# psweens/VAN-GAN

Hardware: AMD Instinct MI355X
Metric: train Mvoxels/s (VanGan.train_step, 128^3 bf16) (higher is better)
Workload: dtype bf16; 1 GPU; VanGan.train_step, 128x128x128 volumes, batch 1 per GPU (global 1), clDice on, disc noise+dropout on; parallelism=dp1

## Files before the change

van_gan_amd/csrc/vg_c1k3.hip:

```cpp
#include "vg_c1k3.h"

namespace {
constexpr int TW = 16, TD = 4;
constexpr int ROWB = TW * 8 + 8;

typedef __attribute__((ext_vector_type(2))) unsigned u32x2;
typedef __attribute__((ext_vector_type(4))) unsigned u32x4;
typedef __attribute__((ext_vector_type(4))) short s16x4;
typedef __attribute__((ext_vector_type(2))) float f32x2;

template <int KS, int ST, int TH> struct Geo {
    static constexpr int IH = ST * TH + KS - ST, ID = ST * TD + KS - ST;
    static constexpr int NROWS = ID * IH, IMGB = NROWS * ROWB;
    static constexpr int NI = 3 * ST + 4;
    static constexpr int NRT = KS * KS;
};

__device__ __forceinline__ float c1_slope(int act) { return act == VG_ACT_RELU ? 0.f : (act == VG_ACT_LRELU ? VG_LRELU : 1.f); }

template <typename S, int KS, int ST, int TH, bool NOISE>
__device__ __forceinline__ void c1_stage_image(const C1M& p, char* img, int n, int od0, int oh0, int ow0, float sc, float sf, float slope, int tid) {
    typedef Geo<KS, ST, TH> G;
    const bool refl = p.pad_mode == VG_PAD_REFLECT;
    for (int item = tid; item < G::NROWS * 4; item += 256) {
        const int row = item >> 2, q = item & 3;
        const int zz = row / G::IH, yy = row - zz * G::IH;
        const int pd = ST * od0 + p.td0 + zz, ph = ST * oh0 + p.th0 + yy, pw0 = ST * (ow0 + 4 * q) + p.tw0;
        bool okd, okh;
        const int rd = c1_resolve(pd, p.D, refl, okd), rh = c1_resolve(ph, p.H, refl, okh);
        const S* src = (const S*)p.x + (((int64_t)n * p.D + rd) * p.H + rh) * p.W;
        const bf16_t* nz = nullptr;
        if (NOISE) nz = (const bf16_t*)p.noise + (((int64_t)n * (p.D + 2) + min(max(pd + 1, 0), p.D + 1)) * (p.H + 2) + min(max(ph + 1, 0), p.H + 1)) * (p.W + 2);
        float v[G::NI], nv[G::NI]; bool ok[G::NI];
#pragma unroll
        for (int i = 0; i < G::NI; ++i) {
            const int cw = c1_resolve(pw0 + i, p.W, refl, ok[i]);
            v[i] = ld_global(src + cw);
            nv[i] = NOISE ? ld_global(nz + min(max(pw0 + i + 1, 0), p.W + 1)) : 0.f;
        }
        unsigned short h[G::NI];
#pragma unroll
        for (int i = 0; i < G::NI; ++i) {
            float y = v[i] * sc + sf;
            y = fmaxf(y, y * slope);
            y = (okd && okh && ok[i]) ? y : 0.f;
            h[i] = f2bf(y + nv[i]);
        }
        char* dst = img + row * ROWB + q * 32;
#pragma unroll
        for (int e = 0; e < 4; ++e)
            *(u32x2*)(dst + e * 8) = (u32x2){h[ST * e] | ((unsigned)h[ST * e + 1] << 16), h[ST * e + 2] | ((unsigned)h[ST * e + 3] << 16)};
    }
}

template <int KS>
__device__ __forceinline__ bf16x8 c1_weight_frag(const C1M& p, int co, int kg, int s) {
    bf16x8 r;
#pragma unroll
    for (int i = 0; i < 8; ++i) {
        const int k = 32 * s + 8 * kg + i, t = k >> 2, j = k & 3;
        r[i] = (t < KS * KS && j < KS) ? (short)((const bf16_t*)p.w)[(size_t)co * p.Ktot + t * p.CK + j] : (short)0;
    }
    return r;
}

template <typename S, int KS, int ST, int MT, bool NOISE>
__global__ __launch_bounds__(256, 2) void c1m_fwd_kernel(const C1M p) {
    typedef bf16_t T;
    constexpr int TH = 8, C = 16 * MT;
    typedef Geo<KS, ST, TH> G;
    __shared__ __attribute__((aligned(16))) char img[G::IMGB];
    __shared__ float stat[32 * MT];
    const int tid = threadIdx.x, lane = tid & 63, wave = __builtin_amdgcn_readfirstlane(tid >> 6);
    const int li = lane & 15, kg = lane >> 4;
    const int n = blockIdx.y;
    const float sc = p.scale ? p.scale[n] : p.sc, sf = p.scale ? p.shift[n] : p.sf, slope = c1_slope(p.act);
    bf16x8 wa[MT][2];
    f32x2 eb[MT][2];
#pragma unroll
    for (int mt = 0; mt < MT; ++mt) {
        wa[mt][0] = c1_weight_frag<KS>(p, 16 * mt + li, kg, 0); wa[mt][1] = c1_weight_frag<KS>(p, 16 * mt + li, kg, 1);
        const int c = 16 * mt + 4 * kg;
        eb[mt][0] = (f32x2){0.f, 0.f}; eb[mt][1] = eb[mt][0];
        if (p.bias) { eb[mt][0] = (f32x2){p.bias[c], p.bias[c + 1]}; eb[mt][1] = (f32x2){p.bias[c + 2], p.bias[c + 3]}; }
    }
    if (tid < 32 * MT) stat[tid] = 0.f;
    int boff[2][2];
#pragma unroll
    for (int s = 0; s < 2; ++s)
#pragma unroll
        for (int h = 0; h < 2; ++h) {
            const int t = min(8 * s + 2 * kg + h, G::NRT - 1), a = t / KS, b = t - a * KS;
            boff[s][h] = ((ST * wave + a) * G::IH + b) * ROWB + li * 8;
        }
    const int tiles_w = (p.OW + TW - 1) / TW, tiles_h = (p.OH + TH - 1) / TH, tiles_d = (p.OD + TD - 1) / TD;
    const int ntiles = tiles_w * tiles_h * tiles_d;
    float s1[MT][4], s2[MT][4];
#pragma unroll
    for (int mt = 0; mt < MT; ++mt)
#pragma unroll
        for (int r = 0; r < 4; ++r) { s1[mt][r] = 0.f; s2[mt][r] = 0.f; }
    const int cst = 8 * (kg >> 1), jodd = kg & 1;
    const size_t rowpitch = (size_t)p.OW * C;
    for (int tile = blockIdx.x; tile < ntiles; tile += gridDim.x) {
        const int tw = tile % tiles_w, t2 = tile / tiles_w, th = t2 % tiles_h, td = t2 / tiles_h;
        const int od0 = td * TD, oh0 = th * TH, ow0 = tw * TW;
        __syncthreads();
        c1_stage_image<S, KS, ST, TH, NOISE>(p, img, n, od0, oh0, ow0, sc, sf, slope, tid);
        __syncthreads();
        const int od = od0 + wave, ow = ow0 + li;
        const bool dw_ok = od < p.OD && ow < p.OW;
        T* const obase = (T*)p.out + ((((size_t)n * p.OD + min(od, p.OD - 1)) * p.OH + oh0) * p.OW + min(ow, p.OW - 1)) * C + cst;
#pragma unroll
        for (int mt = 0; mt < MT; ++mt) {
            f32x4 acc[8];
#pragma unroll
            for (int j = 0; j < 8; ++j) {
                const int jo = ST * j * ROWB;
                const u32x2 a0 = *(const u32x2*)(img + boff[0][0] + jo), a1 = *(const u32x2*)(img + boff[0][1] + jo);
                const u32x2 c0 = *(const u32x2*)(img + boff[1][0] + jo), c1 = *(const u32x2*)(img + boff[1][1] + jo);
                const bf16x8 b0 = __builtin_bit_cast(bf16x8, ((u32x4){a0[0], a0[1], a1[0], a1[1]}));
                const bf16x8 b1 = __builtin_bit_cast(bf16x8, ((u32x4){c0[0], c0[1], c1[0], c1[1]}));
                acc[j] = VG_MFMA16(wa[mt][0], b0, ((f32x4){0.f, 0.f, 0.f, 0.f}));
                acc[j] = VG_MFMA16(wa[mt][1], b1, acc[j]);
            }
            T* const optr = obase + 16 * mt;
#pragma unroll
            for (int jp = 0; jp < 8; jp += 2) {
                bf16x4 pk[2];
#pragma unroll
                for (int e = 0; e < 2; ++e) {
                    const int j = jp + e;
                    const bool ok = dw_ok && oh0 + j < p.OH;
                    f32x2 v0 = {acc[j][0], acc[j][1]}, v1 = {acc[j][2], acc[j][3]};
                    v0 += eb[mt][0]; v1 += eb[mt][1];
                    pk[e] = (bf16x4){(short)f2bf(v0[0]), (short)f2bf(v0[1]), (short)f2bf(v1[0]), (short)f2bf(v1[1])};
                    f32x2 q0 = {bf2f((bf16_t)pk[e][0]), bf2f((bf16_t)pk[e][1])}, q1 = {bf2f((bf16_t)pk[e][2]), bf2f((bf16_t)pk[e][3])};
                    if (!ok) { q0 = (f32x2){0.f, 0.f}; q1 = q0; }
                    s1[mt][0] += q0[0]; s1[mt][1] += q0[1]; s1[mt][2] += q1[0]; s1[mt][3] += q1[1];
                    s2[mt][0] += q0[0] * q0[0]; s2[mt][1] += q0[1] * q0[1]; s2[mt][2] += q1[0] * q1[0]; s2[mt][3] += q1[1] * q1[1];
                }
                const u32x2 wa_ = __builtin_bit_cast(u32x2, pk[0]), wb_ = __builtin_bit_cast(u32x2, pk[1]);
                const u32x2 x0 = __builtin_amdgcn_permlane16_swap(wa_[0], wb_[0], false, false);
                const u32x2 x1 = __builtin_amdgcn_permlane16_swap(wa_[1], wb_[1], false, false);
                const u32x4 outv = {x0[0], x1[0], x0[1], x1[1]};
                const int j = jp + jodd;
                if (dw_ok && oh0 + j < p.OH) *(u32x4*)(optr + j * rowpitch) = outv;
            }
        }
    }
    if (!p.sums) return;
#pragma unroll
    for (int mt = 0; mt < MT; ++mt)
#pragma unroll
        for (int r = 0; r < 4; ++r) {
            float a = s1[mt][r], b = s2[mt][r];
#pragma unroll
            for (int o = 1; o < 16; o <<= 1) { a += __shfl_xor(a, o); b += __shfl_xor(b, o); }
            if (li == 0) { atomicAdd(&stat[(16 * mt + 4 * kg + r) * 2], a); atomicAdd(&stat[(16 * mt + 4 * kg + r) * 2 + 1], b); }
        }
    __syncthreads();
    if (tid < 32 * MT) {
        const int stripe = blockIdx.x & (VG_STRIPES - 1);
        atomicAdd(&p.sums[((size_t)stripe * gridDim.y + n) * (2 * C) + tid], stat[tid]);
    }
    if (p.fin.ticket) vg_fin_tail(p.fin, p.sums, gridDim.y, C, gridDim.x * gridDim.y, (int*)img);
}

template <typename S, int KS, int ST, int TH, int NT, bool NOISE>
__global__ __launch_bounds__(256, 2) void c1m_wgrad_kernel(const C1M p) {
    typedef bf16_t T;
    typedef Geo<KS, ST, TH> G;
    constexpr int C = 16 * NT, VB = 2 * C;
    constexpr int DYROW = TW * VB, DYB = TD * TH * DYROW;
    constexpr int MTS = (G::NRT + 1 + 3) / 4;
    constexpr int UPT = DYB / 16 / 256;
    static_assert(MTS * NT * 1024 <= DYB, "the accumulator exchange reuses the dY tile");
    __shared__ __attribute__((aligned(16))) char img[G::IMGB + 16];
    __shared__ __attribute__((aligned(16))) char dyt[DYB];
    const int tid = threadIdx.x, lane = tid & 63, wave = __builtin_amdgcn_readfirstlane(tid >> 6);
    const int n = blockIdx.y;
    const float sc = p.scale ? p.scale[n] : p.sc, sf = p.scale ? p.shift[n] : p.sf, slope = c1_slope(p.act);
    if (tid == 0) {
        const unsigned one = f2bf(1.f);
        *(u32x4*)(img + G::IMGB) = (u32x4){one | (one << 16), one | (one << 16), 0u, 0u};
    }
    const int g = lane >> 4, q = (lane >> 2) & 3, pp = lane & 3;
    const int wq = 8 * (g & 1) + q, yq = g >> 1;
    int aoff[MTS], amove[MTS];
#pragma unroll
    for (int mt = 0; mt < MTS; ++mt) {
        const int r = 4 * mt + pp, a = r / KS, b = r - a * KS;
        amove[mt] = r < G::NRT ? 1 : 0;
        aoff[mt] = r < G::NRT ? ((ST * wave + a) * G::IH + ST * yq + b) * ROWB + wq * 8 : (r == G::NRT ? G::IMGB : G::IMGB + 8);
    }
    const int boff = ((wave * TH + yq) * TW + wq) * VB + pp * 8;
    const int tiles_w = (p.OW + TW - 1) / TW, tiles_h = (p.OH + TH - 1) / TH, tiles_d = (p.OD + TD - 1) / TD;
    const int ntiles = tiles_w * tiles_h * tiles_d;
    f32x4 acc[MTS][NT];
#pragma unroll
    for (int mt = 0; mt < MTS; ++mt)
#pragma unroll
        for (int nt = 0; nt < NT; ++nt) acc[mt][nt] = (f32x4){0.f, 0.f, 0.f, 0.f};
    typedef __attribute__((address_space(3))) s16x4 lds_s4;
    for (int tile = blockIdx.x; tile < ntiles; tile += gridDim.x) {
        const int tw = tile % tiles_w, t2 = tile / tiles_w, th = t2 % tiles_h, td = t2 / tiles_h;
        const int od0 = td * TD, oh0 = th * TH, ow0 = tw * TW;
        f32x4 dv[UPT];
#pragma unroll
        for (int i = 0; i < UPT; ++i) {
            const int u = tid + 256 * i, vox = u / (2 * NT), c16 = u - vox * (2 * NT);
            const int w = vox & 15, y = (vox >> 4) % TH, z = vox / (16 * TH);
            const bool ok = od0 + z < p.OD && oh0 + y < p.OH && ow0 + w < p.OW;
            const T* src = (const T*)p.dy + ((((size_t)n * p.OD + min(od0 + z, p.OD - 1)) * p.OH + min(oh0 + y, p.OH - 1)) * p.OW + min(ow0 + w, p.OW - 1)) * C + c16 * 8;
            dv[i] = *(const __attribute__((address_space(1))) f32x4*)(uintptr_t)src;
            if (!ok) dv[i] = (f32x4){0.f, 0.f, 0.f, 0.f};
        }
        __syncthreads();
        c1_stage_image<S, KS, ST, TH, NOISE>(p, img, n, od0, oh0, ow0, sc, sf, slope, tid);
#pragma unroll
        for (int i = 0; i < UPT; ++i) *(f32x4*)(dyt + (tid + 256 * i) * 16) = dv[i];
        __syncthreads();
#pragma unroll
        for (int s = 0; s < TH / 2; ++s) {
            bf16x8 a[MTS];
#pragma unroll
            for (int mt = 0; mt < MTS; ++mt) {
                const int o = aoff[mt] + amove[mt] * (s * 2 * ST * ROWB);
                const s16x4 lo = __builtin_amdgcn_ds_read_tr16_b64_v4i16((lds_s4*)(img + o));
                const s16x4 hi = __builtin_amdgcn_ds_read_tr16_b64_v4i16((lds_s4*)(img + o + amove[mt] * 32));
                a[mt] = (bf16x8){lo[0], lo[1], lo[2], lo[3], hi[0], hi[1], hi[2], hi[3]};
            }
#pragma unroll
            for (int nt = 0; nt < NT; ++nt) {
                const s16x4 lo = __builtin_amdgcn_ds_read_tr16_b64_v4i16((lds_s4*)(dyt + boff + s * 2 * DYROW + nt * 32));
                const s16x4 hi = __builtin_amdgcn_ds_read_tr16_b64_v4i16((lds_s4*)(dyt + boff + s * 2 * DYROW + nt * 32 + 4 * VB));
                const bf16x8 b = {lo[0], lo[1], lo[2], lo[3], hi[0], hi[1], hi[2], hi[3]};
#pragma unroll
                for (int mt = 0; mt < MTS; ++mt) acc[mt][nt] = VG_MFMA16(a[mt], b, acc[mt][nt]);
            }
        }
    }
    float* red = (float*)dyt;
    __syncthreads();
    for (int i = tid; i < MTS * NT * 256; i += 256) red[i] = 0.f;
    __syncthreads();
#pragma unroll
    for (int mt = 0; mt < MTS; ++mt)
#pragma unroll
        for (int nt = 0; nt < NT; ++nt)
#pragma unroll
            for (int e = 0; e < 4; ++e) atomicAdd(&red[((mt * NT + nt) * 4 + e) * 64 + lane], acc[mt][nt][e]);
    __syncthreads();
    float* slab = p.part ? p.part + ((size_t)blockIdx.y * gridDim.x + blockIdx.x) * (KS * KS * KS * C) : nullptr;
    for (int i = tid; i < MTS * NT * 256; i += 256) {
        const int l = i & 63, e = (i >> 6) & 3, t = i >> 8, nt = t % NT, mt = t / NT;
        const int r = 4 * mt + (l >> 4), co = 16 * nt + (l & 15);
        const float v = red[i];
        if (r < G::NRT && e < KS) {
            const int idx = (r * KS + e) * C + co;
            if (slab) slab[idx] = v; else atomicAdd(&p.dw[idx], v);
        } else if (r == G::NRT && e == 0 && p.db) atomicAdd(&p.db[co], v);
    }
}
}

static bool c1m_fill(const vg_conv_desc* d, C1M& p) {
    if (!vg_tune("C1M", 1) || d->f32 || d->out_f32 || d->c_src0 != 1 || d->src1 || d->c_src1 || d->nclass > 1) return false;
    const int KS = d->wpack;
    if (KS != 3 && KS != 4) return false;
    if (d->istr != KS - 2 || d->ntaps != KS * KS || d->Cout != (KS == 3 ? 16 : 64)) return false;
    for (int t = 0; t < KS * KS; ++t)
        if (d->tap_d[t] != d->tap_d[0] + t / KS || d->tap_h[t] != d->tap_h[0] + t % KS || d->tap_w[t] != 0) return false;
    if (d->noise && !(d->noise_pad == 1 && d->pad_mode == VG_PAD_REFLECT)) return false;
    if (d->D < 2 || d->H < 2 || d->W < 2 || d->OD < 1 || d->OH < 1 || d->OW < 1) return false;
    p = C1M{};
    p.x = d->src0; p.x_f32 = d->src_f32; p.sc = 1.f; p.sf = 0.f; p.scale = d->in_scale; p.shift = d->in_shift; p.act = d->act;
    p.pad_mode = d->pad_mode; p.noise = d->noise;
    p.D = d->D; p.H = d->H; p.W = d->W; p.OD = d->OD; p.OH = d->OH; p.OW = d->OW; p.C = d->Cout;
    p.td0 = d->tap_d[0]; p.th0 = d->tap_h[0]; p.tw0 = d->wpack_wmin;
    p.w = d->wpacked; p.CK = d->CK; p.Ktot = ((KS * KS * d->CK + 31) / 32) * 32;
    return true;
}
static dim3 c1m_grid(const C1M& c, int N, int th, int per_cu) {
    const int64_t tiles = (int64_t)((c.OD + TD - 1) / TD) * ((c.OH + th - 1) / th) * ((c.OW + TW - 1) / TW);
    int64_t b = (int64_t)256 * per_cu / (N > 0 ? N : 1);
    if (b > tiles) b = tiles;
    if (b < 1) b = 1;
    return dim3((unsigned)b, (unsigned)N);
}

template <typename S, int KS, int MT>
static void c1m_launch_fwd(const C1M& c, dim3 grid, hipStream_t s) {
    if (c.noise) hipLaunchKernelGGL((c1m_fwd_kernel<S, KS, KS - 2, MT, true>), grid, dim3(256), 0, s, c);
    else hipLaunchKernelGGL((c1m_fwd_kernel<S, KS, KS - 2, MT, false>), grid, dim3(256), 0, s, c);
}
int c1m_fwd(const vg_conv_desc* d, hipStream_t s) {
    C1M c;
    if (!c1m_fill(d, c)) return 1;
    c.bias = d->bias; c.out = d->out; c.sums = d->out_sums; c.fin = vg_fin_of(d);
    const int KS = d->wpack;
    if (vg_dry("c1m_fwd<%s,%d,%d,%d,n%d>", d->src_f32 ? "f32" : "bf16", KS, KS - 2, c.C / 16, c.noise ? 1 : 0)) return VG_OK;
    const dim3 grid = c1m_grid(c, d->N, 8, vg_tune("C1M_FWD_WGS", KS == 3 ? 4 : 2));
    if (KS == 3) { if (d->src_f32) c1m_launch_fwd<float, 3, 1>(c, grid, s); else c1m_launch_fwd<bf16_t, 3, 1>(c, grid, s); }
    else { if (d->src_f32) c1m_launch_fwd<float, 4, 4>(c, grid, s); else c1m_launch_fwd<bf16_t, 4, 4>(c, grid, s); }
    if (c.sums && c.fin.ticket) vg_fin_done = true;
    return vg_check_launch();
}

template <typename S, int KS, int TH, int NT>
static void c1m_launch_wgrad(const C1M& c, dim3 grid, hipStream_t s) {
    if (c.noise) hipLaunchKernelGGL((c1m_wgrad_kernel<S, KS, KS - 2, TH, NT, true>), grid, dim3(256), 0, s, c);
    else hipLaunchKernelGGL((c1m_wgrad_kernel<S, KS, KS - 2, TH, NT, false>), grid, dim3(256), 0, s, c);
}
int c1m_wgrad(const vg_conv_desc* d, const void* dy, int dy_f32, int T_total, float* dw, float* db, float* scratch, int64_t scratch_bytes, hipStream_t s) {
    C1M c;
    if (dy_f32 || !vg_tune("C1M_WGRAD", 1) || !c1m_fill(d, c)) return 1;
    const int KS = d->wpack;
    if (T_total != KS * KS) return 1;
    c.dy = dy; c.dw = dw; c.db = db;
    const int th = KS == 3 ? 8 : 4;
    const dim3 grid = c1m_grid(c, d->N, th, vg_tune("C1M_WGRAD_WGS", KS == 3 ? 2 : 1));
    const int nslab = (int)(grid.x * grid.y), dw_elems = KS * KS * KS * c.C;
    c.part = (nslab > 4 && scratch && (int64_t)nslab * dw_elems * 4 <= scratch_bytes && vg_tune("C1M_WGRAD_PART", 1)) ? scratch : nullptr;
    if (vg_dry("c1m_wgrad<%s,%d,%d,%d,n%d>|part%d", d->src_f32 ? "f32" : "bf16", KS, KS - 2, c.C / 16, c.noise ? 1 : 0, c.part ? 1 : 0)) return VG_OK;
    if (KS == 3) { if (d->src_f32) c1m_launch_wgrad<float, 3, 8, 1>(c, grid, s); else c1m_launch_wgrad<bf16_t, 3, 8, 1>(c, grid, s); }
    else { if (d->src_f32) c1m_launch_wgrad<float, 4, 4, 4>(c, grid, s); else c1m_launch_wgrad<bf16_t, 4, 4, 4>(c, grid, s); }
    if (c.part) vg_launch_reduce_partials(c.part, nslab, dw_elems, dw, s);
    return vg_check_launch();
}

namespace {
__global__ __launch_bounds__(256) void cell_pack_kernel(const float* __restrict__ w, int C, int Ktot, bf16_t* __restrict__ out) {
    const size_t total = (size_t)64 * Ktot;
    for (size_t i = (size_t)blockIdx.x * 256 + threadIdx.x; i < total; i += (size_t)gridDim.x * 256) {
        const int row = (int)(i / Ktot), k = (int)(i % Ktot);
        const int chunk = k / 448, kl = k % 448, tap = kl / 16, ch = chunk * 16 + (kl & 15);
        float v = 0.f;
        if (row < 8 && tap < 27 && ch < C) {
            const int nd = tap / 9, nh = (tap / 3) % 3, nw = tap % 3;
            const int td = ((row >> 2) & 1) + 2 - 2 * nd, th = ((row >> 1) & 1) + 2 - 2 * nh, tw = (row & 1) + 2 - 2 * nw;
            if (td >= 0 && th >= 0 && tw >= 0) v = w[(size_t)((td * 4 + th) * 4 + tw) * C + ch];
        }
        out[i] = f2bf(v);
    }
}
__global__ __launch_bounds__(256) void cells_fold_kernel(const bf16_t* __restrict__ cells, int D, int H, int W, float* __restrict__ dx) {
    const int n = blockIdx.y;
    const int CD = D / 2 + 1, CH = H / 2 + 1, CW = W / 2 + 1;
    const bf16_t* cb = cells + (size_t)n * CD * CH * CW * 16;
    const int64_t total = (int64_t)D * H * W;
    for (int64_t i = (int64_t)blockIdx.x * 256 + threadIdx.x; i < total; i += (int64_t)gridDim.x * 256) {
        const int iw = (int)(i % W); const int64_t r = i / W; const int ih = (int)(r % H), id = (int)(r / H);
        int pd[2], ph[2], pw[2], nd = 1, nh = 1, nw = 1;
        pd[0] = id + 1; ph[0] = ih + 1; pw[0] = iw + 1;
        if (id == 1) pd[nd++] = 0; else if (id == D - 2) pd[nd++] = D + 1;
        if (ih == 1) ph[nh++] = 0; else if (ih == H - 2) ph[nh++] = H + 1;
        if (iw == 1) pw[nw++] = 0; else if (iw == W - 2) pw[nw++] = W + 1;
        float s = 0.f;
        for (int a = 0; a < nd; ++a)
            for (int b = 0; b < nh; ++b)
                for (int c = 0; c < nw; ++c) {
                    const int qd = pd[a], qh = ph[b], qw = pw[c];
                    s += bf2f(cb[(((size_t)(qd >> 1) * CH + (qh >> 1)) * CW + (qw >> 1)) * 16 + ((qd & 1) * 4 + (qh & 1) * 2 + (qw & 1))]);
                }
        dx[(size_t)n * total + i] = s;
    }
}
}

extern "C" int vg_pack_cell_weights(const float* w, int C, void* out, vg_stream_t stream) {
    vg_begin();
    if (!w || !out || C < 16 || (C % 16)) return VG_EINVAL;
    const int Ktot = (C / 16) * 448;
    hipLaunchKernelGGL(cell_pack_kernel, dim3((64 * Ktot + 255) / 256), dim3(256), 0, (hipStream_t)stream, w, C, Ktot, (bf16_t*)out);
    return vg_check_launch();
}
extern "C" int vg_cells_fold(const void* cells, int N, int D, int H, int W, float* dx, vg_stream_t stream) {
    vg_begin();
    if (!cells || !dx || N < 1 || D < 4 || H < 4 || W < 4 || ((D | H | W) & 1)) return VG_EINVAL;
    int64_t b = ((int64_t)D * H * W + 255) / 256;
    if (b > 2047 / N) b = 2047 / N > 0 ? 2047 / N : 1;
    hipLaunchKernelGGL(cells_fold_kernel, dim3((unsigned)b, (unsigned)N), dim3(256), 0, (hipStream_t)stream, (const bf16_t*)cells, D, H, W, dx);
    return vg_check_launch();
}
```

Measured before the change: 124.2 Mvoxels/s.

## Double-buffer c1m wgrad tiles with async global-to-LDS loads and overlap staging

Adds a pipelined path to the single-channel conv weight-gradient kernel. It double-buffers LDS, issues global-to-LDS DMA for the dY tile and register-held loads for the input image of the next tile, then runs the MFMA work on the current tile. The path is on by default for wgrad; a similar pipelined forward path is added but off by default. The goal is to hide global load latency behind compute, at the cost of doubling LDS and lowering occupancy for the NT=4 variant to one block per CU.

```diff
diff --git a/van_gan_amd/csrc/vg_c1k3.hip b/van_gan_amd/csrc/vg_c1k3.hip
--- a/van_gan_amd/csrc/vg_c1k3.hip
+++ b/van_gan_amd/csrc/vg_c1k3.hip
@@ -1,4 +1,5 @@
 #include "vg_c1k3.h"
+#include "vg_dma_common.h"
 
 namespace {
 constexpr int TW = 16, TD = 4;
@@ -8,6 +9,8 @@
 typedef __attribute__((ext_vector_type(4))) unsigned u32x4;
 typedef __attribute__((ext_vector_type(4))) short s16x4;
 typedef __attribute__((ext_vector_type(2))) float f32x2;
+
+template <int I> using IC = std::integral_constant<int, I>;
 
 template <int KS, int ST, int TH> struct Geo {
     static constexpr int IH = ST * TH + KS - ST, ID = ST * TD + KS - ST;
@@ -53,6 +56,81 @@
     }
 }
 
+__device__ __forceinline__ float c1_ld_raw(const float* p) { return *(const __attribute__((address_space(1))) float*)(uintptr_t)p; }
+__device__ __forceinline__ unsigned c1_ld_raw(const bf16_t* p) { return *(const __attribute__((address_space(1))) bf16_t*)(uintptr_t)p; }
+__device__ __forceinline__ float c1_val(float x) { return x; }
+__device__ __forceinline__ float c1_val(unsigned x) { return bf2f((bf16_t)x); }
+__device__ __forceinline__ int c1_resolve_sel(int p, int n, bool reflect, bool& ok) {
+    const int a = p < 0 ? -p : p, r = a >= n ? 2 * n - 2 - a : a;
+    const bool in = p >= 0 && p < n;
+    ok = reflect || in;
+    return reflect ? min(max(r, 0), n - 1) : (in ? p : 0);
+}
+
+template <typename S, int KS, int ST, int TH, bool NOISE>
+struct C1Stage {
+    typedef Geo<KS, ST, TH> G;
+    static constexpr int ITEMS = (G::NROWS * 4 + 255) / 256;
+    decltype(c1_ld_raw((const S*)nullptr)) v[ITEMS][G::NI];
+    unsigned nv[ITEMS][NOISE ? G::NI : 1];
+    unsigned ok[ITEMS];
+    template <int K0 = 0, int K1 = ITEMS>
+    __device__ __forceinline__ void request(const C1M& p, int n, int od0, int oh0, int ow0, int tid) {
+        const bool refl = p.pad_mode == VG_PAD_REFLECT;
+        asm volatile("" : "+v"(tid));
+#pragma unroll
+        for (int k = K0; k < K1; ++k) {
+            const int item = min(tid + 256 * k, G::NROWS * 4 - 1);
+            const int row = item >> 2, q = item & 3;
+            const int zz = row / G::IH, yy = row - zz * G::IH;
+            const int pd = ST * od0 + p.td0 + zz, ph = ST * oh0 + p.th0 + yy, pw0 = ST * (ow0 + 4 * q) + p.tw0;
+            bool okd, okh;
+            const int rd = c1_resolve_sel(pd, p.D, refl, okd), rh = c1_resolve_sel(ph, p.H, refl, okh);
+            const S* src = (const S*)p.x + (((int64_t)n * p.D + rd) * p.H + rh) * p.W;
+            const bf16_t* nz = nullptr;
+            if (NOISE) nz = (const bf16_t*)p.noise + (((int64_t)n * (p.D + 2) + min(max(pd + 1, 0), p.D + 1)) * (p.H + 2) + min(max(ph + 1, 0), p.H + 1)) * (p.W + 2);
+            unsigned m = 0;
+#pragma unroll
+            for (int i = 0; i < G::NI; ++i) {
+                bool o;
+                const int cw = c1_resolve_sel(pw0 + i, p.W, refl, o);
+                v[k][i] = c1_ld_raw(src + cw);
+                if (NOISE) nv[k][NOISE ? i : 0] = c1_ld_raw(nz + min(max(pw0 + i + 1, 0), p.W + 1));
+                m |= o ? 1u << i : 0u;
+            }
+            ok[k] = (okd && okh) ? m : 0u;
+        }
+    }
+    template <int K0 = 0, int K1 = ITEMS>
+    __device__ __forceinline__ void commit(char* img, float sc, float sf, float slope, int tid) const {
+        asm volatile("" : "+v"(tid));
+#pragma unroll
+        for (int k = K0; k < K1; ++k) {
+            const int item = tid + 256 * k;
+            const int row = item >> 2, q = item & 3;
+            unsigned short h[G::NI];
+#pragma unroll
+            for (int i = 0; i < G::NI; ++i) {
+                float y = c1_val(v[k][i]) * sc + sf;
+                y = fmaxf(y, y * slope);
+                y = ((ok[k] >> i) & 1u) ? y : 0.f;
+                h[i] = f2bf(y + (NOISE ? bf2f(nv[k][NOISE ? i : 0]) : 0.f));
+            }
+            char* dst = img + row * ROWB + q * 32;
+            u32x2 ent[4];
+#pragma unroll
+            for (int e = 0; e < 4; ++e) {
+                ent[e] = (u32x2){h[ST * e] | ((unsigned)h[ST * e + 1] << 16), h[ST * e + 2] | ((unsigned)h[ST * e + 3] << 16)};
+                asm volatile("" : "+v"(ent[e]));
+            }
+            if (item < G::NROWS * 4) {
+#pragma unroll
+                for (int e = 0; e < 4; ++e) *(u32x2*)(dst + e * 8) = ent[e];
+            }
+        }
+    }
+};
+
 template <int KS>
 __device__ __forceinline__ bf16x8 c1_weight_frag(const C1M& p, int co, int kg, int s) {
     bf16x8 r;
@@ -64,13 +142,13 @@
     return r;
 }
 
-template <typename S, int KS, int ST, int MT, bool NOISE>
+template <typename S, int KS, int ST, int MT, bool NOISE, bool PIPE>
 __global__ __launch_bounds__(256, 2) void c1m_fwd_kernel(const C1M p) {
     typedef bf16_t T;
     constexpr int TH = 8, C = 16 * MT;
     typedef Geo<KS, ST, TH> G;
-    __shared__ __attribute__((aligned(16))) char img[G::IMGB];
-    __shared__ float stat[32 * MT];
+    __shared__ __attribute__((aligned(16))) char smem[(PIPE ? 2 : 1) * G::IMGB + 32 * MT * 4];
+    float* const stat = (float*)(smem + (PIPE ? 2 : 1) * G::IMGB);
     const int tid = threadIdx.x, lane = tid & 63, wave = __builtin_amdgcn_readfirstlane(tid >> 6);
     const int li = lane & 15, kg = lane >> 4;
     const int n = blockIdx.y;
@@ -102,17 +180,12 @@
         for (int r = 0; r < 4; ++r) { s1[mt][r] = 0.f; s2[mt][r] = 0.f; }
     const int cst = 8 * (kg >> 1), jodd = kg & 1;
     const size_t rowpitch = (size_t)p.OW * C;
-    for (int tile = blockIdx.x; tile < ntiles; tile += gridDim.x) {
-        const int tw = tile % tiles_w, t2 = tile / tiles_w, th = t2 % tiles_h, td = t2 / tiles_h;
-        const int od0 = td * TD, oh0 = th * TH, ow0 = tw * TW;
-        __syncthreads();
-        c1_stage_image<S, KS, ST, TH, NOISE>(p, img, n, od0, oh0, ow0, sc, sf, slope, tid);
-        __syncthreads();
+    auto multiply = [&](const char* img, int od0, int oh0, int ow0, auto MT0, auto MT1) {
         const int od = od0 + wave, ow = ow0 + li;
         const bool dw_ok = od < p.OD && ow < p.OW;
         T* const obase = (T*)p.out + ((((size_t)n * p.OD + min(od, p.OD - 1)) * p.OH + oh0) * p.OW + min(ow, p.OW - 1)) * C + cst;
 #pragma unroll
-        for (int mt = 0; mt < MT; ++mt) {
+        for (int mt = decltype(MT0)::value; mt < decltype(MT1)::value; ++mt) {
             f32x4 acc[8];
 #pragma unroll
             for (int j = 0; j < 8; ++j) {
@@ -148,6 +221,63 @@
                 if (dw_ok && oh0 + j < p.OH) *(u32x4*)(optr + j * rowpitch) = outv;
             }
         }
+    };
+    if constexpr (PIPE) {
+        const int ntw = (int)blockIdx.x < ntiles ? (ntiles - (int)blockIdx.x + (int)gridDim.x - 1) / (int)gridDim.x : 0;
+        C1Stage<S, KS, ST, TH, NOISE> st;
+        constexpr bool SPLIT = C1Stage<S, KS, ST, TH, NOISE>::ITEMS == 3 && MT == 4;
+        if (ntw > 0) {
+            const int tile = blockIdx.x, tw = tile % tiles_w, t2 = tile / tiles_w, th = t2 % tiles_h, td = t2 / tiles_h;
+            if constexpr (SPLIT) {
+                st.template request<0, 1>(p, n, td * TD, th * TH, tw * TW, tid); st.template commit<0, 1>(smem, sc, sf, slope, tid);
+                st.template request<1, 2>(p, n, td * TD, th * TH, tw * TW, tid); st.template commit<1, 2>(smem, sc, sf, slope, tid);
+                st.template request<2, 3>(p, n, td * TD, th * TH, tw * TW, tid); st.template commit<2, 3>(smem, sc, sf, slope, tid);
+            } else {
+                st.request(p, n, td * TD, th * TH, tw * TW, tid);
+                st.commit(smem, sc, sf, slope, tid);
+            }
+        }
+#pragma unroll
+        for (int mt = 0; mt < MT; ++mt) asm volatile("" : "+v"(wa[mt][0]), "+v"(wa[mt][1]), "+v"(eb[mt][0]), "+v"(eb[mt][1]));
+        __syncthreads();
+        for (int it = 0; it + 1 < ntw; ++it) {
+            const int tile = blockIdx.x + it * gridDim.x;
+            const int tw = tile % tiles_w, t2 = tile / tiles_w, th = t2 % tiles_h, td = t2 / tiles_h;
+            const int tn = tile + gridDim.x, twn = tn % tiles_w, t2n = tn / tiles_w, thn = t2n % tiles_h, tdn = t2n / tiles_h;
+            const char* img = smem + (it & 1) * G::IMGB;
+            char* nxt = smem + ((it + 1) & 1) * G::IMGB;
+            if constexpr (SPLIT) {
+                st.template request<0, 1>(p, n, tdn * TD, thn * TH, twn * TW, tid);
+                multiply(img, td * TD, th * TH, tw * TW, IC<0>(), IC<1>());
+                st.template commit<0, 1>(nxt, sc, sf, slope, tid);
+                st.template request<1, 2>(p, n, tdn * TD, thn * TH, twn * TW, tid);
+                multiply(img, td * TD, th * TH, tw * TW, IC<1>(), IC<2>());
+                st.template commit<1, 2>(nxt, sc, sf, slope, tid);
+                st.template request<2, 3>(p, n, tdn * TD, thn * TH, twn * TW, tid);
+                multiply(img, td * TD, th * TH, tw * TW, IC<2>(), IC<3>());
+                st.template commit<2, 3>(nxt, sc, sf, slope, tid);
+                multiply(img, td * TD, th * TH, tw * TW, IC<3>(), IC<MT>());
+            } else {
+                st.request(p, n, tdn * TD, thn * TH, twn * TW, tid);
+                multiply(img, td * TD, th * TH, tw * TW, IC<0>(), IC<MT>());
+                st.commit(nxt, sc, sf, slope, tid);
+            }
+            __syncthreads();
+        }
+        if (ntw > 0) {
+            const int tile = blockIdx.x + (ntw - 1) * gridDim.x;
+            const int tw = tile % tiles_w, t2 = tile / tiles_w, th = t2 % tiles_h, td = t2 / tiles_h;
+            multiply(smem + ((ntw - 1) & 1) * G::IMGB, td * TD, th * TH, tw * TW, IC<0>(), IC<MT>());
+        }
+    } else {
+        for (int tile = blockIdx.x; tile < ntiles; tile += gridDim.x) {
+            const int tw = tile % tiles_w, t2 = tile / tiles_w, th = t2 % tiles_h, td = t2 / tiles_h;
+            const int od0 = td * TD, oh0 = th * TH, ow0 = tw * TW;
+            __syncthreads();
+            c1_stage_image<S, KS, ST, TH, NOISE>(p, smem, n, od0, oh0, ow0, sc, sf, slope, tid);
+            __syncthreads();
+            multiply(smem, od0, oh0, ow0, IC<0>(), IC<MT>());
+        }
     }
     if (!p.sums) return;
 #pragma unroll
@@ -164,26 +294,29 @@
         const int stripe = blockIdx.x & (VG_STRIPES - 1);
         atomicAdd(&p.sums[((size_t)stripe * gridDim.y + n) * (2 * C) + tid], stat[tid]);
     }
-    if (p.fin.ticket) vg_fin_tail(p.fin, p.sums, gridDim.y, C, gridDim.x * gridDim.y, (int*)img);
-}
-
-template <typename S, int KS, int ST, int TH, int NT, bool NOISE>
-__global__ __launch_bounds__(256, 2) void c1m_wgrad_kernel(const C1M p) {
+    if (p.fin.ticket) vg_fin_tail(p.fin, p.sums, gridDim.y, C, gridDim.x * gridDim.y, (int*)smem);
+}
+
+template <typename S, int KS, int ST, int TH, int NT, bool NOISE, bool PIPE>
+__global__ __launch_bounds__(256, (PIPE && NT == 4) ? 1 : 2) void c1m_wgrad_kernel(const C1M p) {
     typedef bf16_t T;
     typedef Geo<KS, ST, TH> G;
     constexpr int C = 16 * NT, VB = 2 * C;
     constexpr int DYROW = TW * VB, DYB = TD * TH * DYROW;
     constexpr int MTS = (G::NRT + 1 + 3) / 4;
     constexpr int UPT = DYB / 16 / 256;
+    constexpr int IMGS = G::IMGB + 16;
+    constexpr int NBUF = PIPE ? 2 : 1;
     static_assert(MTS * NT * 1024 <= DYB, "the accumulator exchange reuses the dY tile");
-    __shared__ __attribute__((aligned(16))) char img[G::IMGB + 16];
-    __shared__ __attribute__((aligned(16))) char dyt[DYB];
+    static_assert(IMGS % 16 == 0 && DYB % 4096 == 0, "16-byte units; a wave's DMA piece is 1 KB");
+    __shared__ __attribute__((aligned(16))) char smem[NBUF * (DYB + IMGS)];
+    char* const dyt0 = smem, * const img0 = smem + NBUF * DYB;
     const int tid = threadIdx.x, lane = tid & 63, wave = __builtin_amdgcn_readfirstlane(tid >> 6);
     const int n = blockIdx.y;
     const float sc = p.scale ? p.scale[n] : p.sc, sf = p.scale ? p.shift[n] : p.sf, slope = c1_slope(p.act);
-    if (tid == 0) {
+    if (tid < NBUF) {
         const unsigned one = f2bf(1.f);
-        *(u32x4*)(img + G::IMGB) = (u32x4){one | (one << 16), one | (one << 16), 0u, 0u};
+        *(u32x4*)(img0 + tid * IMGS + G::IMGB) = (u32x4){one | (one << 16), one | (one << 16), 0u, 0u};
     }
     const int g = lane >> 4, q = (lane >> 2) & 3, pp = lane & 3;
     const int wq = 8 * (g & 1) + q, yq = g >> 1;
@@ -203,24 +336,7 @@
 #pragma unroll
         for (int nt = 0; nt < NT; ++nt) acc[mt][nt] = (f32x4){0.f, 0.f, 0.f, 0.f};
     typedef __attribute__((address_space(3))) s16x4 lds_s4;
-    for (int tile = blockIdx.x; tile < ntiles; tile += gridDim.x) {
-        const int tw = tile % tiles_w, t2 = tile / tiles_w, th = t2 % tiles_h, td = t2 / tiles_h;
-        const int od0 = td * TD, oh0 = th * TH, ow0 = tw * TW;
-        f32x4 dv[UPT];
-#pragma unroll
-        for (int i = 0; i < UPT; ++i) {
-            const int u = tid + 256 * i, vox = u / (2 * NT), c16 = u - vox * (2 * NT);
-            const int w = vox & 15, y = (vox >> 4) % TH, z = vox / (16 * TH);
-            const bool ok = od0 + z < p.OD && oh0 + y < p.OH && ow0 + w < p.OW;
-            const T* src = (const T*)p.dy + ((((size_t)n * p.OD + min(od0 + z, p.OD - 1)) * p.OH + min(oh0 + y, p.OH - 1)) * p.OW + min(ow0 + w, p.OW - 1)) * C + c16 * 8;
-            dv[i] = *(const __attribute__((address_space(1))) f32x4*)(uintptr_t)src;
-            if (!ok) dv[i] = (f32x4){0.f, 0.f, 0.f, 0.f};
-        }
-        __syncthreads();
-        c1_stage_image<S, KS, ST, TH, NOISE>(p, img, n, od0, oh0, ow0, sc, sf, slope, tid);
-#pragma unroll
-        for (int i = 0; i < UPT; ++i) *(f32x4*)(dyt + (tid + 256 * i) * 16) = dv[i];
-        __syncthreads();
+    auto multiply = [&](const char* img, const char* dyt) {
 #pragma unroll
         for (int s = 0; s < TH / 2; ++s) {
             bf16x8 a[MTS];
@@ -240,8 +356,69 @@
                 for (int mt = 0; mt < MTS; ++mt) acc[mt][nt] = VG_MFMA16(a[mt], b, acc[mt][nt]);
             }
         }
-    }
-    float* red = (float*)dyt;
+    };
+    if constexpr (PIPE) {
+        const int ntw = (int)blockIdx.x < ntiles ? (ntiles - (int)blockIdx.x + (int)gridDim.x - 1) / (int)gridDim.x : 0;
+        const char* const dyn = (const char*)p.dy + (size_t)n * p.OD * p.OH * p.OW * VB;
+        const unsigned lds0 = (unsigned)(uintptr_t)(lds_void_d*)smem;
+        C1Stage<S, KS, ST, TH, NOISE> st;
+        auto request = [&](int tile, int buf) -> unsigned {
+            const int tw = tile % tiles_w, t2 = tile / tiles_w, th = t2 % tiles_h, td = t2 / tiles_h;
+            const int od0 = td * TD, oh0 = th * TH, ow0 = tw * TW;
+            const unsigned ldsb = __builtin_amdgcn_readfirstlane(lds0 + buf * DYB + wave * 1024);
+            unsigned outside = 0;
+#pragma unroll
+            for (int i = 0; i < UPT; ++i) {
+                const int u = tid + 256 * i, vox = u / (2 * NT), c16 = u - vox * (2 * NT);
+                const int w = vox & 15, y = (vox >> 4) % TH, z = vox / (16 * TH);
+                const bool ok = od0 + z < p.OD && oh0 + y < p.OH && ow0 + w < p.OW;
+                const int off = (((min(od0 + z, p.OD - 1) * p.OH + min(oh0 + y, p.OH - 1)) * p.OW + min(ow0 + w, p.OW - 1)) * C + c16 * 8) * 2;
+                glds16(dyn, off, ldsb + i * 4096);
+                outside |= ok ? 0u : 1u << i;
+            }
+            st.request(p, n, od0, oh0, ow0, tid);
+            return outside;
+        };
+        auto commit = [&](int buf, unsigned outside) {
+            st.commit(img0 + buf * IMGS, sc, sf, slope, tid);
+            asm volatile("s_waitcnt vmcnt(0)" ::: "memory");
+#pragma unroll
+            for (int i = 0; i < UPT; ++i)
+                if ((outside >> i) & 1u) *(f32x4*)(dyt0 + buf * DYB + (tid + 256 * i) * 16) = (f32x4){0.f, 0.f, 0.f, 0.f};
+        };
+        if (ntw > 0) { const unsigned o = request(blockIdx.x, 0); commit(0, o); }
+        __syncthreads();
+        for (int it = 0; it + 1 < ntw; ++it) {
+            const int cur = it & 1;
+            const unsigned outside = request(blockIdx.x + (it + 1) * gridDim.x, cur ^ 1);
+            multiply(img0 + cur * IMGS, dyt0 + cur * DYB);
+            commit(cur ^ 1, outside);
+            __syncthreads();
+        }
+        if (ntw > 0) multiply(img0 + ((ntw - 1) & 1) * IMGS, dyt0 + ((ntw - 1) & 1) * DYB);
+    } else {
+        for (int tile = blockIdx.x; tile < ntiles; tile += gridDim.x) {
+            const int tw = tile % tiles_w, t2 = tile / tiles_w, th = t2 % tiles_h, td = t2 / tiles_h;
+            const int od0 = td * TD, oh0 = th * TH, ow0 = tw * TW;
+            f32x4 dv[UPT];
+#pragma unroll
+            for (int i = 0; i < UPT; ++i) {
+                const int u = tid + 256 * i, vox = u / (2 * NT), c16 = u - vox * (2 * NT);
+                const int w = vox & 15, y = (vox >> 4) % TH, z = vox / (16 * TH);
+                const bool ok = od0 + z < p.OD && oh0 + y < p.OH && ow0 + w < p.OW;
+                const T* src = (const T*)p.dy + ((((size_t)n * p.OD + min(od0 + z, p.OD - 1)) * p.OH + min(oh0 + y, p.OH - 1)) * p.OW + min(ow0 + w, p.OW - 1)) * C + c16 * 8;
+                dv[i] = *(const __attribute__((address_space(1))) f32x4*)(uintptr_t)src;
+                if (!ok) dv[i] = (f32x4){0.f, 0.f, 0.f, 0.f};
+            }
+            __syncthreads();
+            c1_stage_image<S, KS, ST, TH, NOISE>(p, img0, n, od0, oh0, ow0, sc, sf, slope, tid);
+#pragma unroll
+            for (int i = 0; i < UPT; ++i) *(f32x4*)(dyt0 + (tid + 256 * i) * 16) = dv[i];
+            __syncthreads();
+            multiply(img0, dyt0);
+        }
+    }
+    float* red = (float*)dyt0;
     __syncthreads();
     for (int i = tid; i < MTS * NT * 256; i += 256) red[i] = 0.f;
     __syncthreads();
@@ -286,14 +463,20 @@
     const int64_t tiles = (int64_t)((c.OD + TD - 1) / TD) * ((c.OH + th - 1) / th) * ((c.OW + TW - 1) / TW);
     int64_t b = (int64_t)256 * per_cu / (N > 0 ? N : 1);
     if (b > tiles) b = tiles;
+    const int cap = vg_tune("C1M_MAX_WGS", 0);
+    if (cap > 0 && b > cap) b = cap;
     if (b < 1) b = 1;
     return dim3((unsigned)b, (unsigned)N);
 }
 
+template <typename S, int KS, int MT, bool PIPE>
+static void c1m_launch_fwd(const C1M& c, dim3 grid, hipStream_t s) {
+    if (c.noise) hipLaunchKernelGGL((c1m_fwd_kernel<S, KS, KS - 2, MT, true, PIPE>), grid, dim3(256), 0, s, c);
+    else hipLaunchKernelGGL((c1m_fwd_kernel<S, KS, KS - 2, MT, false, PIPE>), grid, dim3(256), 0, s, c);
+}
 template <typename S, int KS, int MT>
-static void c1m_launch_fwd(const C1M& c, dim3 grid, hipStream_t s) {
-    if (c.noise) hipLaunchKernelGGL((c1m_fwd_kernel<S, KS, KS - 2, MT, true>), grid, dim3(256), 0, s, c);
-    else hipLaunchKernelGGL((c1m_fwd_kernel<S, KS, KS - 2, MT, false>), grid, dim3(256), 0, s, c);
+static void c1m_launch_fwd(const C1M& c, dim3 grid, bool pipe, hipStream_t s) {
+    if (pipe) c1m_launch_fwd<S, KS, MT, true>(c, grid, s); else c1m_launch_fwd<S, KS, MT, false>(c, grid, s);
 }
 int c1m_fwd(const vg_conv_desc* d, hipStream_t s) {
     C1M c;
@@ -302,16 +485,21 @@
     const int KS = d->wpack;
     if (vg_dry("c1m_fwd<%s,%d,%d,%d,n%d>", d->src_f32 ? "f32" : "bf16", KS, KS - 2, c.C / 16, c.noise ? 1 : 0)) return VG_OK;
     const dim3 grid = c1m_grid(c, d->N, 8, vg_tune("C1M_FWD_WGS", KS == 3 ? 4 : 2));
-    if (KS == 3) { if (d->src_f32) c1m_launch_fwd<float, 3, 1>(c, grid, s); else c1m_launch_fwd<bf16_t, 3, 1>(c, grid, s); }
-    else { if (d->src_f32) c1m_launch_fwd<float, 4, 4>(c, grid, s); else c1m_launch_fwd<bf16_t, 4, 4>(c, grid, s); }
+    const bool pipe = vg_tune("C1M_PIPE", 1) != 0 && vg_tune("C1M_PIPE_FWD", 0) != 0;
+    if (KS == 3) { if (d->src_f32) c1m_launch_fwd<float, 3, 1>(c, grid, pipe, s); else c1m_launch_fwd<bf16_t, 3, 1>(c, grid, pipe, s); }
+    else { if (d->src_f32) c1m_launch_fwd<float, 4, 4>(c, grid, pipe, s); else c1m_launch_fwd<bf16_t, 4, 4>(c, grid, pipe, s); }
     if (c.sums && c.fin.ticket) vg_fin_done = true;
     return vg_check_launch();
 }
 
+template <typename S, int KS, int TH, int NT, bool PIPE>
+static void c1m_launch_wgrad(const C1M& c, dim3 grid, hipStream_t s) {
+    if (c.noise) hipLaunchKernelGGL((c1m_wgrad_kernel<S, KS, KS - 2, TH, NT, true, PIPE>), grid, dim3(256), 0, s, c);
+    else hipLaunchKernelGGL((c1m_wgrad_kernel<S, KS, KS - 2, TH, NT, false, PIPE>), grid, dim3(256), 0, s, c);
+}
 template <typename S, int KS, int TH, int NT>
-static void c1m_launch_wgrad(const C1M& c, dim3 grid, hipStream_t s) {
-    if (c.noise) hipLaunchKernelGGL((c1m_wgrad_kernel<S, KS, KS - 2, TH, NT, true>), grid, dim3(256), 0, s, c);
-    else hipLaunchKernelGGL((c1m_wgrad_kernel<S, KS, KS - 2, TH, NT, false>), grid, dim3(256), 0, s, c);
+static void c1m_launch_wgrad(const C1M& c, dim3 grid, bool pipe, hipStream_t s) {
+    if (pipe) c1m_launch_wgrad<S, KS, TH, NT, true>(c, grid, s); else c1m_launch_wgrad<S, KS, TH, NT, false>(c, grid, s);
 }
 int c1m_wgrad(const vg_conv_desc* d, const void* dy, int dy_f32, int T_total, float* dw, float* db, float* scratch, int64_t scratch_bytes, hipStream_t s) {
     C1M c;
@@ -324,8 +512,9 @@
     const int nslab = (int)(grid.x * grid.y), dw_elems = KS * KS * KS * c.C;
     c.part = (nslab > 4 && scratch && (int64_t)nslab * dw_elems * 4 <= scratch_bytes && vg_tune("C1M_WGRAD_PART", 1)) ? scratch : nullptr;
     if (vg_dry("c1m_wgrad<%s,%d,%d,%d,n%d>|part%d", d->src_f32 ? "f32" : "bf16", KS, KS - 2, c.C / 16, c.noise ? 1 : 0, c.part ? 1 : 0)) return VG_OK;
-    if (KS == 3) { if (d->src_f32) c1m_launch_wgrad<float, 3, 8, 1>(c, grid, s); else c1m_launch_wgrad<bf16_t, 3, 8, 1>(c, grid, s); }
-    else { if (d->src_f32) c1m_launch_wgrad<float, 4, 4, 4>(c, grid, s); else c1m_launch_wgrad<bf16_t, 4, 4, 4>(c, grid, s); }
+    const bool pipe = vg_tune("C1M_PIPE", 1) != 0 && (int64_t)c.OD * c.OH * c.OW * c.C * 2 < ((int64_t)1 << 31);
+    if (KS == 3) { if (d->src_f32) c1m_launch_wgrad<float, 3, 8, 1>(c, grid, pipe, s); else c1m_launch_wgrad<bf16_t, 3, 8, 1>(c, grid, pipe, s); }
+    else { if (d->src_f32) c1m_launch_wgrad<float, 4, 4, 4>(c, grid, pipe, s); else c1m_launch_wgrad<bf16_t, 4, 4, 4>(c, grid, pipe, s); }
     if (c.part) vg_launch_reduce_partials(c.part, nslab, dw_elems, dw, s);
     return vg_check_launch();
 }
```

Measured after the change: 124.7 Mvoxels/s (median of 6 runs). No clear change (+0.4%).
